# CompVis/behavior-driven-video-synthesis

Hardware: AMD Instinct MI355X
Metric: frames/sec VUnet 256x256 bs=16 fwd+bwd (higher is better)
Workload: dtype f32 (operands scaled by a power of two and split into 2 fp16 terms, 3 partial products on fp16 MFMA, fp32 accumulate; weight gradients and uncovered layers: 3 bf16 terms / 6 products, fp32-input MFMA, fp32 VALU); 1 GPU; Human3.6m shape_and_pose_net VunetAlter 256x256 per-GPU bs=16 fwd+bwd, VGG19 perceptual + KL loss, fused Adam, dropout 0.05, regressor side loop off, seeded-synthetic VGG19 weights, rasterised synthetic stickmen; global_batch=16, parallelism=dp1, conv_precision=h2, hip_streams=4, hip_graph=True, graph_settle_steps=7, rccl_world_size=1, dp_backend=none

## Files before the change

### behavior_driven_video_synthesis_amd/csrc/conv_wgrad_h2.hip

```cpp
#include <type_traits>

#include "common.h"
#include "split_h2.h"

typedef h2_f16x8 wg_bf16x8;
typedef uint32_t wg_u32x4 __attribute__((ext_vector_type(4)));
typedef float wg_f32x4 __attribute__((ext_vector_type(4)));

#ifdef WG_TSTAMP
static __device__ unsigned long long wg_ts[4096 * 16];
#define WG_STAMP(k_)                                                                                                     \
  do {                                                                                                                   \
    if (lane == 0 && wave == 0 && step == (nsteps >> 1)) {                                                                           \
      const unsigned b_ = (blockIdx.z * gridDim.y + blockIdx.y) * gridDim.x + blockIdx.x;                                \
      if (b_ < 4096) wg_ts[b_ * 16 + grp * 8 + (k_)] = __builtin_amdgcn_s_memrealtime();                                 \
    }                                                                                                                    \
  } while (0)
extern "C" int WG_TSTAMP(unsigned long long* out, int nblocks) {
  return hipMemcpyFromSymbol(out, HIP_SYMBOL(wg_ts), sizeof(unsigned long long) * 16 * (size_t)nblocks) == hipSuccess ? 0 : -1;
}
#define WG_STAMP_AT(slot_)                                                                                               \
  do {                                                                                                                   \
    if (threadIdx.x == 0) {                                                                                              \
      const unsigned b_ = (blockIdx.z * gridDim.y + blockIdx.y) * gridDim.x + blockIdx.x;                                \
      if (b_ < 4096) wg_ts[b_ * 16 + (slot_)] = __builtin_amdgcn_s_memrealtime();                                        \
    }                                                                                                                    \
  } while (0)
#else
#define WG_STAMP(k_)
#define WG_STAMP_AT(slot_)
#endif

__device__ __forceinline__ void wg_dma4(const void* gsrc, uint32_t lds_addr) {
  uint32_t keep;
  asm volatile("s_mov_b32 %0, m0\n\ts_mov_b32 m0, %2\n\ts_nop 0\n\tglobal_load_lds_dword %1, off\n\ts_mov_b32 m0, %0"
               : "=&s"(keep)
               : "v"(gsrc), "s"(lds_addr)
               : "memory");
}

struct WgradH2Args {
  vunet_wgrad_desc d;
  const float* x1;
  const float* x2;
  const float* dy;
  float* slabs;
  float* dshift;
  int Ctot, Coutp, tiles_per_img_w, tiles_per_img, ntiles, tps;
  InAct in1, in2;
  const float* amax_x;
  const float* amax_x2;
  const float* amax_dy;
};

constexpr int WG_GROUPS = 2;

template <int MTW>
__global__ __launch_bounds__(256 * WG_GROUPS, 1) void conv_wgrad_h2_kernel(const WgradH2Args a_in) {
  WgradH2Args a = a_in;
  WG_STAMP_AT(7);
  inact_resolve(a.in1);
  inact_resolve(a.in2);
  constexpr int TH = 4;
  constexpr int WP = 4 / MTW;
  constexpr int RW = TH / WP;
  constexpr int ENT = 6 * 32;
  constexpr int PL = ENT * 5 + 1;
  constexpr int EPL = 6 * 4 * 32;
  constexpr bool DMA = MTW == 1;
  constexpr int SU = 2 * PL + 2 * EPL / 4;
  constexpr int RU = ENT * 8 + 2 * ENT / 4;
  constexpr int GU = SU + (DMA ? RU : 0);
  constexpr int G = WG_GROUPS;
  extern __shared__ __attribute__((aligned(16))) uint4 smem4[];

  const vunet_wgrad_desc& d = a.d;
  const int grp = threadIdx.x >> 8;
  const int tid = threadIdx.x & 255, lane = tid & 63, wave = tid >> 6;
  wg_u32x4* const xL = reinterpret_cast<wg_u32x4*>(smem4 + grp * GU);
  uint32_t* const eL = reinterpret_cast<uint32_t*>(smem4 + grp * GU + 2 * PL);
  const wg_f32x4* const rawL = reinterpret_cast<const wg_f32x4*>(smem4 + grp * GU + SU);
  const float* const haloL = reinterpret_cast<const float*>(smem4 + grp * GU + SU + ENT * 8);
  const int j = lane & 31, h = lane >> 5;
  const int wm = wave / WP, pw = wave % WP;
  const int split = blockIdx.x;
  const int ci0 = blockIdx.y * 32;
  const int co0 = blockIdx.z * 32 * MTW;
  const int H = d.Hs, W = d.Ws;

  float sx, sdy, descale, descale2;
  {
    const float4 px = h2_amax4(a.amax_x, a.amax_x2, tid), pd = reinterpret_cast<const float4*>(a.amax_dy)[tid];
    float mx = wave_max(fmaxf(fmaxf(px.x, px.y), fmaxf(px.z, px.w)));
    float md = wave_max(fmaxf(fmaxf(pd.x, pd.y), fmaxf(pd.z, pd.w)));
    float* const redm = reinterpret_cast<float*>(smem4) + grp * 8;
    if (lane == 0) { redm[wave] = mx; redm[4 + wave] = md; }
    __syncthreads();
    mx = fmaxf(fmaxf(redm[0], redm[1]), fmaxf(redm[2], redm[3]));
    md = fmaxf(fmaxf(redm[4], redm[5]), fmaxf(redm[6], redm[7]));
    __syncthreads();
    if (a.in1.thresh) mx *= a.in1.keep_scale;
    const int ex = h2_scale_exp(mx), ed = h2_scale_exp(md);
    sx = h2_pow2(ex);
    sdy = h2_pow2(ed);
    h2_pow2_pair(-(ex + ed), descale, descale2);
  }

  const bool second = ci0 >= d.C1;
  const float* __restrict__ xs = second ? a.x2 : a.x1;
  const int Cs = second ? d.C2 : d.C1;
  const int cbase = second ? ci0 - d.C1 : ci0;
  InAct ia = a.in1;
  ia.seed = second ? a.in2.seed : a.in1.seed;

  f32x16 acc[9];
#pragma unroll
  for (int t = 0; t < 9; ++t)
#pragma unroll
    for (int r = 0; r < 16; ++r) acc[t][r] = 0.f;
  float dsum = 0.f;

  int s_row[3], s_ci[3], s_oct[3];
#pragma unroll
  for (int i = 0; i < 3; ++i) {
    const int u = tid + 256 * i;
    s_oct[i] = u & 3;
    s_ci[i] = (u >> 2) & 31;
    s_row[i] = u >> 7;
  }
  const int co_lane = co0 + wm * 32 + j;

  const int t_begin = split * a.tps;
  const int t_end = min(t_begin + a.tps, a.ntiles);

  wg_f32x4 xv[3][2];
  float hv[2];
  uint32_t gidx[3], hidx = 0;
  uint32_t okbits = 0;
  auto tile_origin = [&](int tile, int& n, int& row0, int& col0) {
    n = tile / a.tiles_per_img;
    const int tr = tile - n * a.tiles_per_img;
    const int ty = tr / a.tiles_per_img_w, tx = tr - ty * a.tiles_per_img_w;
    row0 = ty * TH;
    col0 = tx * 32;
  };
  auto issue_x = [&](int tile) {
    int n, row0, col0;
    tile_origin(tile, n, row0, col0);
    okbits = 0;
#pragma unroll
    for (int i = 0; i < 3; ++i) {
      const int ih = row0 - 1 + s_row[i];
      const bool ok = (unsigned)ih < (unsigned)H;
      okbits |= (ok ? 1u : 0u) << i;
      gidx[i] = (uint32_t)(((n * Cs + cbase + s_ci[i]) * H + (ok ? ih : 0)) * W + col0 + 8 * s_oct[i]);
      xv[i][0] = *reinterpret_cast<const wg_f32x4*>(xs + gidx[i]);
      xv[i][1] = *reinterpret_cast<const wg_f32x4*>(xs + gidx[i] + 4);
    }
    {
      const int e = tid < ENT ? tid : tid - 64;
      const int r = e >> 5, c = e & 31;
      const int ih = row0 - 1 + r;
      const bool rok = (unsigned)ih < (unsigned)H;
      hidx = (uint32_t)(((n * Cs + cbase + c) * H + (rok ? ih : 0)) * W + col0);
      const bool okl = rok && col0 > 0, okr = rok && col0 + 32 < W;
      okbits |= (okl ? 16u : 0u) | (okr ? 32u : 0u);
      hv[0] = xs[okl ? hidx - 1 : hidx];
      hv[1] = xs[okr ? hidx + 32 : hidx];
    }
  };
  const int wave_u = __builtin_amdgcn_readfirstlane(wave);
  const uint32_t raw_addr = (uint32_t)__builtin_amdgcn_readfirstlane(
      (int)(uint32_t)(uintptr_t)(__attribute__((address_space(3))) void*)(smem4 + grp * GU + SU));
  auto dma_x = [&](int tile) {
    int n, row0, col0;
    tile_origin(tile, n, row0, col0);
#pragma unroll
    for (int i = 0; i < 3; ++i) {
      const int ih = row0 - 1 + s_row[i];
      const bool ok = (unsigned)ih < (unsigned)H;
      const float* src = xs + (size_t)((n * Cs + cbase + s_ci[i]) * H + (ok ? ih : 0)) * W + col0 + 8 * s_oct[i];
      h2_dma16(src, raw_addr + (uint32_t)(((wave_u * 3 + i) * 2 + 0) * 64) * 16u);
      h2_dma16(src + 4, raw_addr + (uint32_t)(((wave_u * 3 + i) * 2 + 1) * 64) * 16u);
    }
    if (wave_u < 3) {
      const int ih = row0 - 1 + (tid >> 5);
      const bool rok = (unsigned)ih < (unsigned)H;
      const float* base = xs + (size_t)((n * Cs + cbase + (tid & 31)) * H + (rok ? ih : 0)) * W + col0;
      wg_dma4(base + ((rok && col0 > 0) ? -1 : 0), raw_addr + (uint32_t)(ENT * 8) * 16u + (uint32_t)(wave_u * 64) * 4u);
      wg_dma4(base + ((rok && col0 + 32 < W) ? 32 : 0), raw_addr + (uint32_t)(ENT * 8) * 16u + (uint32_t)(ENT + wave_u * 64) * 4u);
    }
  };
  int f_n = 0, f_row0 = 0, f_col0 = 0;
  auto fetch_unit = [&](int i) {
    const int ih = f_row0 - 1 + s_row[i];
    const bool ok = (unsigned)ih < (unsigned)H;
    okbits = (okbits & ~(1u << i)) | ((ok ? 1u : 0u) << i);
    gidx[i] = (uint32_t)(((f_n * Cs + cbase + s_ci[i]) * H + (ok ? ih : 0)) * W + f_col0 + 8 * s_oct[i]);
    xv[i][0] = rawL[((wave * 3 + i) * 2 + 0) * 64 + lane];
    xv[i][1] = rawL[((wave * 3 + i) * 2 + 1) * 64 + lane];
  };
  auto fetch_halo = [&]() {
    const int e = tid < ENT ? tid : tid - 64;
    const int r = e >> 5, c = e & 31;
    const int ih = f_row0 - 1 + r;
    const bool rok = (unsigned)ih < (unsigned)H;
    hidx = (uint32_t)(((f_n * Cs + cbase + c) * H + (rok ? ih : 0)) * W + f_col0);
    const bool okl = rok && f_col0 > 0, okr = rok && f_col0 + 32 < W;
    okbits = (okbits & 7u) | (okl ? 16u : 0u) | (okr ? 32u : 0u);
    hv[0] = haloL[e];
    hv[1] = haloL[ENT + e];
  };
  auto write_x_as = [&](auto pro_c, auto from_lds_c) {
    constexpr int PRO = decltype(pro_c)::value;
    constexpr bool FROM_LDS = decltype(from_lds_c)::value;
#pragma unroll
    for (int i = 0; i < 3; ++i) {
      if constexpr (FROM_LDS) fetch_unit(i);
      const bool ok = (okbits >> i) & 1u;
      const float sxk = ok ? sx : 0.f;
      float f[8];
#pragma unroll
      for (int e = 0; e < 8; ++e) {
        const float t = e < 4 ? xv[i][0][e] : xv[i][1][e - 4];
        f[e] = in_act_form<PRO>(ia, ok ? t : 0.f, gidx[i] + e) * sxk;
      }
      uint32_t ph[4], pl[4];
      h2_split2_nat(f[0], f[1], ph[0], pl[0]);
      h2_split2_nat(f[2], f[3], ph[1], pl[1]);
      h2_split2_nat(f[4], f[5], ph[2], pl[2]);
      h2_split2_nat(f[6], f[7], ph[3], pl[3]);
      const int unit = (s_row[i] * 32 + s_ci[i]) * 5 + 1 + s_oct[i];
      xL[unit] = wg_u32x4{ph[0], ph[1], ph[2], ph[3]};
      xL[PL + unit] = wg_u32x4{pl[0], pl[1], pl[2], pl[3]};
      unsigned short* const eb = reinterpret_cast<unsigned short*>(eL);
      const int e0 = (s_row[i] * 4 + s_oct[i]) * 32 + s_ci[i];
      if (s_oct[i] > 0) {
        eb[2 * (e0 - 32)] = (unsigned short)(ph[0] & 0xffffu);
        eb[2 * (EPL + e0 - 32)] = (unsigned short)(pl[0] & 0xffffu);
      }
      if (s_oct[i] < 3) {
        eb[2 * (e0 + 32) + 1] = (unsigned short)(ph[3] >> 16);
        eb[2 * (EPL + e0 + 32) + 1] = (unsigned short)(pl[3] >> 16);
      }
    }
    if constexpr (FROM_LDS) fetch_halo();
    if (tid < ENT) {
      const bool okl = okbits & 16u, okr = okbits & 32u;
      const float fl = in_act_form<PRO>(ia, okl ? hv[0] : 0.f, hidx - 1) * (okl ? sx : 0.f);
      const float fr = in_act_form<PRO>(ia, okr ? hv[1] : 0.f, hidx + 32) * (okr ? sx : 0.f);
      uint32_t ph, pl;
      h2_split2_nat(fr, fl, ph, pl);
      unsigned short* const eb = reinterpret_cast<unsigned short*>(eL);
      const int r = tid >> 5, c = tid & 31;
      eb[2 * ((r * 4 + 0) * 32 + c) + 1] = (unsigned short)(ph >> 16);
      eb[2 * (EPL + (r * 4 + 0) * 32 + c) + 1] = (unsigned short)(pl >> 16);
      eb[2 * ((r * 4 + 3) * 32 + c)] = (unsigned short)(ph & 0xffffu);
      eb[2 * (EPL + (r * 4 + 3) * 32 + c)] = (unsigned short)(pl & 0xffffu);
    }
  };
  const int pro_form = in_act_form_of(ia);
  auto write_x = [&]() {
    constexpr std::integral_constant<bool, DMA> from_lds{};
    if (pro_form == 2) write_x_as(std::integral_constant<int, 2>{}, from_lds);
    else if (pro_form == 1) write_x_as(std::integral_constant<int, 1>{}, from_lds);
    else if (pro_form == 0) write_x_as(std::integral_constant<int, 0>{}, from_lds);
    else write_x_as(std::integral_constant<int, 3>{}, from_lds);
  };

  wg_f32x4 dyv[RW][2][2];
  const wg_u32x4* const xl_lane = xL + (pw * RW * 32 + j) * 5 + 1 + h;
  const uint32_t* const el_lane = eL + (pw * RW * 4 + h) * 32 + j;
  const int nsteps = (t_end - t_begin + G - 1) / G;
  auto load_dy = [&](int tile) {
    int n, row0, col0;
    tile_origin(tile, n, row0, col0);
    const float* __restrict__ dp = a.dy + ((size_t)(n * d.Cout + co_lane) * H + row0 + pw * RW) * W + col0 + 8 * h;
#pragma unroll
    for (int rr = 0; rr < RW; ++rr)
#pragma unroll
      for (int s = 0; s < 2; ++s) {
        dyv[rr][s][0] = *reinterpret_cast<const wg_f32x4*>(dp + rr * W + 16 * s);
        dyv[rr][s][1] = *reinterpret_cast<const wg_f32x4*>(dp + rr * W + 16 * s + 4);
      }
  };
  if constexpr (DMA) {
    if (t_begin + grp < t_end) dma_x(t_begin + grp);
  }
  if (G == 2 && grp == 1) __syncthreads();
  for (int step = 0; step < nsteps; ++step) {
    const int mtile = t_begin + step * G + grp;
    const bool valid = mtile < t_end;
    const bool more = mtile + G < t_end;
    WG_STAMP(0);
    if (valid) {
      if constexpr (DMA) {
        asm volatile("s_waitcnt vmcnt(0)" ::: "memory");
        load_dy(mtile);
        tile_origin(mtile, f_n, f_row0, f_col0);
      } else {
        issue_x(mtile);
#ifdef WG_TSTAMP
        asm volatile("s_waitcnt vmcnt(0)" ::: "memory");
#endif
      }
      WG_STAMP(1);
      write_x();
      if constexpr (DMA) {
        asm volatile("s_waitcnt lgkmcnt(0)" : "+v"(dyv[RW - 1][1][1]) :: "memory");
        if (more) dma_x(mtile + G);
      }
    }
    WG_STAMP(2);
    __syncthreads();
    WG_STAMP(3);
    if (valid) {
    if constexpr (!DMA) load_dy(mtile);
#ifdef WG_TSTAMP
    if constexpr (!DMA) asm volatile("s_waitcnt vmcnt(0)" ::: "memory");
    WG_STAMP(4);
#endif

    struct Raw {
      wg_u32x4 c[2];
      uint32_t e[2];
    };
    auto load_raw = [&](int st) {
      const int rr = st / 6, s = (st / 3) & 1, kh = st % 3;
      Raw r;
#pragma unroll
      for (int p = 0; p < 2; ++p) {
        r.c[p] = xl_lane[p * PL + (rr + kh) * 160 + 2 * s];
        r.e[p] = el_lane[p * EPL + ((rr + kh) * 4 + 2 * s) * 32];
      }
      return r;
    };
    constexpr int NSTEP = RW * 6;
    Raw cur = load_raw(0);
    wg_bf16x8 Ah, Al;
#pragma unroll
    for (int st = 0; st < NSTEP; ++st) {
      const int rr = st / 6, s = (st / 3) & 1, kh = st % 3;
      __builtin_amdgcn_sched_barrier(0);
      Raw nxt = cur;
      if (st + 1 < NSTEP) nxt = load_raw(st + 1);
      __builtin_amdgcn_sched_barrier(0);
      if (kh == 0) {
        const wg_f32x4 d0 = dyv[rr][s][0], d1 = dyv[rr][s][1];
        dsum += ((d0[0] + d0[1]) + (d0[2] + d0[3])) + ((d1[0] + d1[1]) + (d1[2] + d1[3]));
        uint32_t ah[4], al[4];
        h2_split2_nat(d0[0] * sdy, d0[1] * sdy, ah[0], al[0]);
        h2_split2_nat(d0[2] * sdy, d0[3] * sdy, ah[1], al[1]);
        h2_split2_nat(d1[0] * sdy, d1[1] * sdy, ah[2], al[2]);
        h2_split2_nat(d1[2] * sdy, d1[3] * sdy, ah[3], al[3]);
        Ah = h2_frag(ah[0], ah[1], ah[2], ah[3]);
        Al = h2_frag(al[0], al[1], al[2], al[3]);
      }
#pragma unroll
      for (int pp = 0; pp < 2; ++pp) {
        const int p = 1 - pp;
        const wg_u32x4 c = cur.c[p];
        const uint32_t s01 = __builtin_amdgcn_alignbit(c.y, c.x, 16), s12 = __builtin_amdgcn_alignbit(c.z, c.y, 16),
                       s23 = __builtin_amdgcn_alignbit(c.w, c.z, 16);
        wg_bf16x8 B[3];
        B[0] = h2_frag(__builtin_amdgcn_alignbit(c.x, cur.e[p], 16), s01, s12, s23);
        B[1] = __builtin_bit_cast(wg_bf16x8, c);
        B[2] = h2_frag(s01, s12, s23, __builtin_amdgcn_alignbit(cur.e[p], c.w, 16));
#pragma unroll
        for (int kw = 0; kw < 3; ++kw) {
          f32x16 cc = acc[kh * 3 + kw];
          if (p == 0) cc = __builtin_amdgcn_mfma_f32_32x32x16_f16(Al, B[kw], cc, 0, 0, 0);
          cc = __builtin_amdgcn_mfma_f32_32x32x16_f16(Ah, B[kw], cc, 0, 0, 0);
          acc[kh * 3 + kw] = cc;
        }
      }
      cur = nxt;
    }
    WG_STAMP(5);
    }
    __syncthreads();
    WG_STAMP(6);
  }
  if (G == 2 && grp == 0) __syncthreads();
  WG_STAMP_AT(15);

  {
    float* const red = reinterpret_cast<float*>(smem4);
    const bool owner = pw == 0 && grp == 0;
    auto fold = [&](auto tc) {
      constexpr int t = decltype(tc)::value;
      __syncthreads();
      if (!owner) {
#pragma unroll
        for (int r = 0; r < 16; ++r) red[((grp * 4 + wave) * 16 + r) * 64 + lane] = acc[t][r];
      }
      __syncthreads();
      if (owner) {
#pragma unroll 1
        for (int pi = 1; pi < G * WP; ++pi) {
          const int src = (pi / WP) * 4 + wave + pi % WP;
#pragma unroll
          for (int r = 0; r < 16; ++r) acc[t][r] += red[(src * 16 + r) * 64 + lane];
        }
      }
    };
    fold(std::integral_constant<int, 0>{});
    fold(std::integral_constant<int, 1>{});
    fold(std::integral_constant<int, 2>{});
    fold(std::integral_constant<int, 3>{});
    fold(std::integral_constant<int, 4>{});
    fold(std::integral_constant<int, 5>{});
    fold(std::integral_constant<int, 6>{});
    fold(std::integral_constant<int, 7>{});
    fold(std::integral_constant<int, 8>{});
    __syncthreads();
    if (!owner) red[(grp * 4 + wave) * 64 + lane] = dsum;
    __syncthreads();
    if (owner)
      for (int g2 = 0; g2 < G; ++g2)
        for (int o = (g2 == 0 ? 1 : 0); o < WP; ++o) dsum += red[(g2 * 4 + wave + o) * 64 + lane];
  }

  const size_t KT = (size_t)9 * a.Ctot;
  float* slab = a.slabs + (size_t)split * a.Coutp * KT;
  const int ci = ci0 + j;
  if (pw == 0 && grp == 0) {
    auto store = [&](auto tc) {
      constexpr int t = decltype(tc)::value;
#pragma unroll
      for (int r = 0; r < 16; ++r) {
        const int co = co0 + wm * 32 + (r & 3) + 8 * (r >> 2) + 4 * h;
        slab[(size_t)co * KT + (size_t)t * a.Ctot + ci] = acc[t][r] * descale * descale2;
      }
    };
    store(std::integral_constant<int, 0>{});
    store(std::integral_constant<int, 1>{});
    store(std::integral_constant<int, 2>{});
    store(std::integral_constant<int, 3>{});
    store(std::integral_constant<int, 4>{});
    store(std::integral_constant<int, 5>{});
    store(std::integral_constant<int, 6>{});
    store(std::integral_constant<int, 7>{});
    store(std::integral_constant<int, 8>{});
    if (blockIdx.y == 0) {
      const float tot = dsum + __shfl_xor(dsum, 32, 64);
      if (h == 0) a.dshift[(size_t)split * a.Coutp + co_lane] = tot;
    }
  }
  WG_STAMP_AT(14);
}

static void h2_geometry(const vunet_wgrad_desc* d, int& MTW, int& ntiles, int& ciblocks, int& coblocks) {
  MTW = d->Cout % 64 == 0 ? 2 : 1;
  ntiles = d->N * (d->Ho / 4) * (d->Wo / 32);
  ciblocks = (d->C1 + d->C2) / 32;
  coblocks = (d->Cout + 32 * MTW - 1) / (32 * MTW);
}

int vunet_wgrad_h2_name(const vunet_wgrad_desc* d, char* name, int len) {
  return snprintf(name, len, "conv_wgrad_h2_kernel<%d>", d->Cout % 64 == 0 ? 2 : 1);
}

int vunet_wgrad_h2_launch(const vunet_wgrad_desc* d, const float* x1, const float* x2, const float* dy, float* slabs,
                          float* dshift, const float* amax_x, const float* amax_x2, const float* amax_dy, hipStream_t st) {
  WgradH2Args a;
  a.d = *d;
  a.x1 = x1; a.x2 = x2; a.dy = dy; a.slabs = slabs; a.dshift = dshift;
  a.amax_x = amax_x; a.amax_x2 = amax_x2; a.amax_dy = amax_dy;
  int MTW, ciblocks, coblocks;
  h2_geometry(d, MTW, a.ntiles, ciblocks, coblocks);
  a.Ctot = d->C1 + d->C2;
  a.Coutp = (d->Cout + 31) / 32 * 32;
  a.tiles_per_img_w = d->Wo / 32;
  a.tiles_per_img = (d->Ho / 4) * a.tiles_per_img_w;
  a.tps = (a.ntiles + d->nsplit - 1) / d->nsplit;
  a.in1 = make_inact(d->in_act, d->in_slope, d->drop_p, d->drop_seed);
  a.in2 = make_inact(d->in_act, d->in_slope, d->drop_p, d->drop_seed + 0x9E3779B9u);
  dim3 grid(d->nsplit, ciblocks, coblocks);
  constexpr size_t staged = (size_t)2 * (6 * 32 * 5 + 1) * 16 + (size_t)2 * 6 * 4 * 32 * 4;
  constexpr size_t raw_bytes = (size_t)6 * 32 * 8 * 16 + (size_t)2 * 6 * 32 * 4;
  constexpr size_t lds1 = WG_GROUPS * (staged + raw_bytes), lds2 = WG_GROUPS * staged;
  static const bool attr_ok = [] {
    return (lds1 <= 64 * 1024 || hipFuncSetAttribute((const void*)conv_wgrad_h2_kernel<1>,
                                                     hipFuncAttributeMaxDynamicSharedMemorySize, (int)lds1) == hipSuccess) &&
           (lds2 <= 64 * 1024 || hipFuncSetAttribute((const void*)conv_wgrad_h2_kernel<2>,
                                                     hipFuncAttributeMaxDynamicSharedMemorySize, (int)lds2) == hipSuccess);
  }();
  if (!attr_ok) return VUNET_ERR_LAUNCH;
  if (MTW == 1) VUNET_LAUNCH((conv_wgrad_h2_kernel<1>), grid, dim3(256 * WG_GROUPS), lds1, st, a);
  else VUNET_LAUNCH((conv_wgrad_h2_kernel<2>), grid, dim3(256 * WG_GROUPS), lds2, st, a);
  return vunet_check_launch();
}
```

Measured before the change: 783.2 frames/s.

## Walk wgrad tiles column-major per group and reuse overlapping halo rows in LDS

Tile order changes from row-major to column-major, going down the image. Each of the two groups in a block now takes a contiguous range of tiles instead of interleaving them. Consecutive tiles in a group are vertically adjacent, so the two halo rows already split and staged in LDS are copied forward and only the new rows are loaded, converted and written. This cuts global loads and fp16 split arithmetic. Split indices are also permuted across blocks, which changes how work is spread across XCDs or caches. The cost is extra LDS copy traffic, more complex fresh/reuse logic, and a risk of wrong halo edges.

```diff
diff --git a/behavior_driven_video_synthesis_amd/csrc/conv_wgrad_h2.hip b/behavior_driven_video_synthesis_amd/csrc/conv_wgrad_h2.hip
--- a/behavior_driven_video_synthesis_amd/csrc/conv_wgrad_h2.hip
+++ b/behavior_driven_video_synthesis_amd/csrc/conv_wgrad_h2.hip
@@ -46,7 +46,7 @@
   const float* dy;
   float* slabs;
   float* dshift;
-  int Ctot, Coutp, tiles_per_img_w, tiles_per_img, ntiles, tps;
+  int Ctot, Coutp, tiles_per_img_w, tiles_per_col, ntiles, tps;
   InAct in1, in2;
   const float* amax_x;
   const float* amax_x2;
@@ -83,7 +83,8 @@
   const float* const haloL = reinterpret_cast<const float*>(smem4 + grp * GU + SU + ENT * 8);
   const int j = lane & 31, h = lane >> 5;
   const int wm = wave / WP, pw = wave % WP;
-  const int split = blockIdx.x;
+  const int nsp = (int)gridDim.x;
+  const int split = nsp % 8 == 0 ? (int)(blockIdx.x % 8) * (nsp / 8) + (int)(blockIdx.x / 8) : (int)blockIdx.x;
   const int ci0 = blockIdx.y * 32;
   const int co0 = blockIdx.z * 32 * MTW;
   const int H = d.Hs, W = d.Ws;
@@ -131,25 +132,40 @@
   const int co_lane = co0 + wm * 32 + j;
 
   const int t_begin = split * a.tps;
-  const int t_end = min(t_begin + a.tps, a.ntiles);
+  const int t_len = max(min(t_begin + a.tps, a.ntiles) - t_begin, 0);
+  const int nsteps = (t_len + G - 1) / G;
+  const int grp_u = __builtin_amdgcn_readfirstlane(grp);
+  const int g_begin = t_begin + min(grp_u * nsteps, t_len);
+  const int g_end = t_begin + min((grp_u + 1) * nsteps, t_len);
+  struct TileAt {
+    int n, tx, ty;
+  };
+  auto tile_at = [&](int tile) {
+    TileAt t;
+    const int col = tile / a.tiles_per_col;
+    t.ty = tile - col * a.tiles_per_col;
+    t.n = col / a.tiles_per_img_w;
+    t.tx = col - t.n * a.tiles_per_img_w;
+    return t;
+  };
+  auto tile_below = [&](TileAt t) {
+    if (++t.ty == a.tiles_per_col) {
+      t.ty = 0;
+      if (++t.tx == a.tiles_per_img_w) t.tx = 0, ++t.n;
+    }
+    return t;
+  };
 
   wg_f32x4 xv[3][2];
   float hv[2];
   uint32_t gidx[3], hidx = 0;
   uint32_t okbits = 0;
-  auto tile_origin = [&](int tile, int& n, int& row0, int& col0) {
-    n = tile / a.tiles_per_img;
-    const int tr = tile - n * a.tiles_per_img;
-    const int ty = tr / a.tiles_per_img_w, tx = tr - ty * a.tiles_per_img_w;
-    row0 = ty * TH;
-    col0 = tx * 32;
-  };
-  auto issue_x = [&](int tile) {
-    int n, row0, col0;
-    tile_origin(tile, n, row0, col0);
+  auto issue_x = [&](const TileAt& t, bool fresh) {
+    const int n = t.n, row0 = t.ty * TH, col0 = t.tx * 32;
     okbits = 0;
 #pragma unroll
     for (int i = 0; i < 3; ++i) {
+      if (i == 0 && !fresh) continue;
       const int ih = row0 - 1 + s_row[i];
       const bool ok = (unsigned)ih < (unsigned)H;
       okbits |= (ok ? 1u : 0u) << i;
@@ -172,18 +188,18 @@
   const int wave_u = __builtin_amdgcn_readfirstlane(wave);
   const uint32_t raw_addr = (uint32_t)__builtin_amdgcn_readfirstlane(
       (int)(uint32_t)(uintptr_t)(__attribute__((address_space(3))) void*)(smem4 + grp * GU + SU));
-  auto dma_x = [&](int tile) {
-    int n, row0, col0;
-    tile_origin(tile, n, row0, col0);
+  auto dma_x = [&](const TileAt& t, bool fresh) {
+    const int n = t.n, row0 = t.ty * TH, col0 = t.tx * 32;
 #pragma unroll
     for (int i = 0; i < 3; ++i) {
+      if (i == 0 && !fresh) continue;
       const int ih = row0 - 1 + s_row[i];
       const bool ok = (unsigned)ih < (unsigned)H;
       const float* src = xs + (size_t)((n * Cs + cbase + s_ci[i]) * H + (ok ? ih : 0)) * W + col0 + 8 * s_oct[i];
       h2_dma16(src, raw_addr + (uint32_t)(((wave_u * 3 + i) * 2 + 0) * 64) * 16u);
       h2_dma16(src + 4, raw_addr + (uint32_t)(((wave_u * 3 + i) * 2 + 1) * 64) * 16u);
     }
-    if (wave_u < 3) {
+    if (wave_u < 3 && (fresh || wave_u > 0)) {
       const int ih = row0 - 1 + (tid >> 5);
       const bool rok = (unsigned)ih < (unsigned)H;
       const float* base = xs + (size_t)((n * Cs + cbase + (tid & 31)) * H + (rok ? ih : 0)) * W + col0;
@@ -211,11 +227,40 @@
     hv[0] = haloL[e];
     hv[1] = haloL[ENT + e];
   };
-  auto write_x_as = [&](auto pro_c, auto from_lds_c) {
+  auto reuse_rows = [&]() {
+    constexpr int DU = 4 * 32 * 5, DE = 4 * 4 * 32;
+    unsigned short* const eb = reinterpret_cast<unsigned short*>(eL);
+    int t = tid;
+    asm volatile("" : "+v"(t));
+    const int oct = t & 3, ci = (t >> 2) & 31, row = t >> 7;
+    const int unit = (row * 32 + ci) * 5 + 1 + oct;
+    const int e0 = (row * 4 + oct) * 32 + ci;
+    xL[unit] = xL[unit + DU];
+    xL[PL + unit] = xL[PL + unit + DU];
+    if (oct > 0) {
+      eb[2 * (e0 - 32)] = eb[2 * (e0 - 32 + DE)];
+      eb[2 * (EPL + e0 - 32)] = eb[2 * (EPL + e0 - 32 + DE)];
+    }
+    if (oct < 3) {
+      eb[2 * (e0 + 32) + 1] = eb[2 * (e0 + 32 + DE) + 1];
+      eb[2 * (EPL + e0 + 32) + 1] = eb[2 * (EPL + e0 + 32 + DE) + 1];
+    }
+    if (t >= 128 && t < ENT) {
+      const int r = t >> 5, c = t & 31;
+      const int el = 2 * ((r * 4 + 0) * 32 + c) + 1, er = 2 * ((r * 4 + 3) * 32 + c);
+      eb[el - 2 * DE] = eb[el];
+      eb[2 * EPL + el - 2 * DE] = eb[2 * EPL + el];
+      eb[er - 2 * DE] = eb[er];
+      eb[2 * EPL + er - 2 * DE] = eb[2 * EPL + er];
+    }
+  };
+  auto write_x_as = [&](auto pro_c, auto from_lds_c, bool fresh) {
     constexpr int PRO = decltype(pro_c)::value;
     constexpr bool FROM_LDS = decltype(from_lds_c)::value;
+    unsigned short* const eb = reinterpret_cast<unsigned short*>(eL);
 #pragma unroll
     for (int i = 0; i < 3; ++i) {
+      if (i == 0 && !fresh) continue;
       if constexpr (FROM_LDS) fetch_unit(i);
       const bool ok = (okbits >> i) & 1u;
       const float sxk = ok ? sx : 0.f;
@@ -233,7 +278,6 @@
       const int unit = (s_row[i] * 32 + s_ci[i]) * 5 + 1 + s_oct[i];
       xL[unit] = wg_u32x4{ph[0], ph[1], ph[2], ph[3]};
       xL[PL + unit] = wg_u32x4{pl[0], pl[1], pl[2], pl[3]};
-      unsigned short* const eb = reinterpret_cast<unsigned short*>(eL);
       const int e0 = (s_row[i] * 4 + s_oct[i]) * 32 + s_ci[i];
       if (s_oct[i] > 0) {
         eb[2 * (e0 - 32)] = (unsigned short)(ph[0] & 0xffffu);
@@ -245,13 +289,12 @@
       }
     }
     if constexpr (FROM_LDS) fetch_halo();
-    if (tid < ENT) {
+    if (tid < ENT && (fresh || tid >= 64)) {
       const bool okl = okbits & 16u, okr = okbits & 32u;
       const float fl = in_act_form<PRO>(ia, okl ? hv[0] : 0.f, hidx - 1) * (okl ? sx : 0.f);
       const float fr = in_act_form<PRO>(ia, okr ? hv[1] : 0.f, hidx + 32) * (okr ? sx : 0.f);
       uint32_t ph, pl;
       h2_split2_nat(fr, fl, ph, pl);
-      unsigned short* const eb = reinterpret_cast<unsigned short*>(eL);
       const int r = tid >> 5, c = tid & 31;
       eb[2 * ((r * 4 + 0) * 32 + c) + 1] = (unsigned short)(ph >> 16);
       eb[2 * (EPL + (r * 4 + 0) * 32 + c) + 1] = (unsigned short)(pl >> 16);
@@ -260,21 +303,19 @@
     }
   };
   const int pro_form = in_act_form_of(ia);
-  auto write_x = [&]() {
+  auto write_x = [&](bool fresh) {
     constexpr std::integral_constant<bool, DMA> from_lds{};
-    if (pro_form == 2) write_x_as(std::integral_constant<int, 2>{}, from_lds);
-    else if (pro_form == 1) write_x_as(std::integral_constant<int, 1>{}, from_lds);
-    else if (pro_form == 0) write_x_as(std::integral_constant<int, 0>{}, from_lds);
-    else write_x_as(std::integral_constant<int, 3>{}, from_lds);
+    if (pro_form == 2) write_x_as(std::integral_constant<int, 2>{}, from_lds, fresh);
+    else if (pro_form == 1) write_x_as(std::integral_constant<int, 1>{}, from_lds, fresh);
+    else if (pro_form == 0) write_x_as(std::integral_constant<int, 0>{}, from_lds, fresh);
+    else write_x_as(std::integral_constant<int, 3>{}, from_lds, fresh);
   };
 
   wg_f32x4 dyv[RW][2][2];
   const wg_u32x4* const xl_lane = xL + (pw * RW * 32 + j) * 5 + 1 + h;
   const uint32_t* const el_lane = eL + (pw * RW * 4 + h) * 32 + j;
-  const int nsteps = (t_end - t_begin + G - 1) / G;
-  auto load_dy = [&](int tile) {
-    int n, row0, col0;
-    tile_origin(tile, n, row0, col0);
+  auto load_dy = [&](const TileAt& t) {
+    const int n = t.n, row0 = t.ty * TH, col0 = t.tx * 32;
     const float* __restrict__ dp = a.dy + ((size_t)(n * d.Cout + co_lane) * H + row0 + pw * RW) * W + col0 + 8 * h;
 #pragma unroll
     for (int rr = 0; rr < RW; ++rr)
@@ -285,37 +326,53 @@
       }
   };
   if constexpr (DMA) {
-    if (t_begin + grp < t_end) dma_x(t_begin + grp);
+    if (g_begin < g_end) dma_x(tile_at(g_begin), true);
   }
+  TileAt cur = tile_at(g_begin);
   if (G == 2 && grp == 1) __syncthreads();
   for (int step = 0; step < nsteps; ++step) {
-    const int mtile = t_begin + step * G + grp;
-    const bool valid = mtile < t_end;
-    const bool more = mtile + G < t_end;
+    const int mtile = g_begin + step;
+    const bool valid = mtile < g_end;
+    const bool more = mtile + 1 < g_end;
+    const bool fresh = step == 0 || cur.ty == 0;
+    const TileAt nxt = tile_below(cur);
     WG_STAMP(0);
     if (valid) {
+      if constexpr (!DMA) {
+        int tq = tid;
+        asm volatile("" : "+v"(tq));
+#pragma unroll
+        for (int i = 0; i < 3; ++i) {
+          const int u = tq + 256 * i;
+          s_oct[i] = u & 3;
+          s_ci[i] = (u >> 2) & 31;
+          s_row[i] = u >> 7;
+        }
+      }
       if constexpr (DMA) {
         asm volatile("s_waitcnt vmcnt(0)" ::: "memory");
-        load_dy(mtile);
-        tile_origin(mtile, f_n, f_row0, f_col0);
+        load_dy(cur);
+        f_n = cur.n, f_row0 = cur.ty * TH, f_col0 = cur.tx * 32;
+        if (!fresh) reuse_rows();
       } else {
-        issue_x(mtile);
+        issue_x(cur, fresh);
+        if (!fresh) reuse_rows();
 #ifdef WG_TSTAMP
         asm volatile("s_waitcnt vmcnt(0)" ::: "memory");
 #endif
       }
       WG_STAMP(1);
-      write_x();
+      write_x(fresh);
       if constexpr (DMA) {
         asm volatile("s_waitcnt lgkmcnt(0)" : "+v"(dyv[RW - 1][1][1]) :: "memory");
-        if (more) dma_x(mtile + G);
+        if (more) dma_x(nxt, nxt.ty == 0);
       }
     }
     WG_STAMP(2);
     __syncthreads();
     WG_STAMP(3);
     if (valid) {
-    if constexpr (!DMA) load_dy(mtile);
+    if constexpr (!DMA) load_dy(cur);
 #ifdef WG_TSTAMP
     if constexpr (!DMA) asm volatile("s_waitcnt vmcnt(0)" ::: "memory");
     WG_STAMP(4);
@@ -380,6 +437,7 @@
     }
     __syncthreads();
     WG_STAMP(6);
+    cur = nxt;
   }
   if (G == 2 && grp == 0) __syncthreads();
   WG_STAMP_AT(15);
@@ -472,7 +530,7 @@
   a.Ctot = d->C1 + d->C2;
   a.Coutp = (d->Cout + 31) / 32 * 32;
   a.tiles_per_img_w = d->Wo / 32;
-  a.tiles_per_img = (d->Ho / 4) * a.tiles_per_img_w;
+  a.tiles_per_col = d->Ho / 4;
   a.tps = (a.ntiles + d->nsplit - 1) / d->nsplit;
   a.in1 = make_inact(d->in_act, d->in_slope, d->drop_p, d->drop_seed);
   a.in2 = make_inact(d->in_act, d->in_slope, d->drop_p, d->drop_seed + 0x9E3779B9u);
```

Measured after the change: 788.7 frames/s, median of 6. Within noise of the previous version (+0.7%).
